# Sin3DM/Sin3DM

Hardware: AMD Instinct MI355X
Metric: DDPM-1000 triplane samples/sec @128^2 latent (higher is better)
Workload: dtype f32; 1 GPU; BASELINE configs[1]: 128^2 triplane (H,W,D)=(128,128,128), 128-ch TriplaneUNetModelSmall, DDPM-1000, batch 1 per GPU; a step = 1 denoising step; batch_per_gpu=1, parallelism=1 independent samples, prewarm_steps=150

## Files before the change

### include/sin3dm_hip.h

```cpp
#ifndef SIN3DM_HIP_H
#define SIN3DM_HIP_H

#include <stddef.h>
#include <stdint.h>

#ifdef __cplusplus
extern "C" {
#endif

#define S3D_ABI_VERSION 13
#define S3D_API __attribute__((visibility("default")))

typedef enum {
    S3D_OK = 0,
    S3D_ERR_INVALID = -1,
    S3D_ERR_MISSING = -2,
    S3D_ERR_HIP = -3,
    S3D_ERR_UNSUPPORTED = -4,
    S3D_ERR_INTERNAL = -5
} s3d_status;

S3D_API int s3d_abi_version(void);

S3D_API int s3d_set_option(const char* name, const char* value);
// ... 88 lines not shown
    const float* noise;
    const float* tables;
} s3d_known_region;
S3D_API int s3d_sampler_step_known(const s3d_sampler_args* a, const s3d_known_region* known, void* stream);
S3D_API int s3d_unet_step_film_known(s3d_unet* m, const float* film, int film_stride, int B, int H, int W, int D,
                       const s3d_sampler_args* step, const s3d_known_region* known, float* model_out, void* stream, int carry_flags);
S3D_API int s3d_sampler_renoise(const float* x_prev, const float* noise, const float* known_tables, const int64_t* t, int32_t T,
                       int64_t batch, int64_t per_sample, float* x_t, void* stream);

enum { S3D_MTAB_CX = 0, S3D_MTAB_C0, S3D_MTAB_C1, S3D_MTAB_CN, S3D_MTAB_ROWS };
typedef struct {
    const float* x0_prev;
    const float* tables;
    int32_t order;
} s3d_multistep;
S3D_API int s3d_sampler_step_multistep(const s3d_sampler_args* a, const s3d_multistep* ms, const s3d_known_region* known ,
                       void* stream);
S3D_API int s3d_unet_step_film_multistep(s3d_unet* m, const float* film, int film_stride, int B, int H, int W, int D,
                       const s3d_sampler_args* step, const s3d_multistep* ms, float* model_out, void* stream, int carry_flags);

S3D_API int s3d_op_triplane_conv(const float* const in[3], float* const out[3], int B, int C, int H, int W, int D,
                         int Cout, int ksize, int is_rollout, const float* const weight[3],
                         const float* const bias[3], void* stream);
S3D_API int s3d_op_triplane_norm_silu(const float* const in[3], float* const out[3], int B, int C, int H, int W, int D,
                              const float* const gamma[3], const float* const beta[3], void* stream);
S3D_API int s3d_op_triplane_resample(const float* const in[3], float* const out[3], int B, int C, const int hi[3],
                             const int wi[3], const int ho[3], const int wo[3], int mode, void* stream);
S3D_API int s3d_op_timestep_embed(const float* t, int B, int dim, float* out, void* stream);
S3D_API int s3d_op_triplane_resblock(const float* const in[3], float* const out[3], const float* emb, int B, int C,
                             int Cout, int H, int W, int D, int emb_dim, int use_scale_shift_norm, int is_rollout,
                             const char* const* names, const float* const* tensors, int n_tensors, void* stream);

typedef struct s3d_decoder s3d_decoder;

typedef struct {
    int32_t geo_feat_channels;
    int32_t tex_feat_channels;
    int32_t feat_channel_up;
    int32_t mlp_hidden_channels;
    int32_t mlp_hidden_layers;
    int32_t tex_channels;
} s3d_decoder_cfg;

S3D_API int s3d_decoder_create(const s3d_decoder_cfg* cfg, s3d_decoder** out);
S3D_API int s3d_decoder_create_variant(const s3d_decoder_cfg* cfg, int32_t variant, s3d_decoder** out);
S3D_API int s3d_decoder_out_channels(const s3d_decoder* d);
// ... 216 lines not shown
```

### sin3dm_amd/_lib.py

```python
from __future__ import annotations

import ctypes as C
import os

_HERE = os.path.dirname(os.path.abspath(__file__))
LIB_PATH = os.path.join(_HERE, "libsin3dm_hip.so")

c_fp = C.POINTER(C.c_float)
c_i64p = C.POINTER(C.c_int64)

ABI_VERSION = 13
TAB_ROWS = ("sqrt_recip", "sqrt_recipm1", "coef1", "coef2", "logvar", "acp", "acp_prev")
KTAB_ROWS = ("sqrt_acp_prev", "sqrt_1m_acp_prev", "sqrt_1m_beta", "sqrt_beta")
MTAB_ROWS = ("cx", "c0", "c1", "cn")
STEP_DDPM, STEP_DDIM, STEP_MEAN_ONLY = 0, 1, 2
CARRY_OUT, CARRY_IN = 1, 2
MEAN_START_X, MEAN_EPSILON = 0, 1
ERR_INVALID, ERR_MISSING, ERR_HIP, ERR_UNSUPPORTED, ERR_INTERNAL = -1, -2, -3, -4, -5
MAX_LANES = 16
MESHSDF_MAX_PAIRS = 1 << 27
RENDER_MAX_PAIRS = 1 << 27
RENDER_TILE, RENDER_SUBPIXEL, RENDER_MAX_COORD, RENDER_MAX_GRID = 16, 256, 1 << 20, 4096
IMGFEAT_INCEPTION, IMGFEAT_ALEXNET = 0, 1
RENDER_AMBIENT, RENDER_DIFFUSE = 0.35, 0.65
# ... 62 lines not shown
    "s3d_unet_current_lane": (C.c_int, [C.c_void_p]),
    "s3d_unet_forward_film": (C.c_int, [C.c_void_p, C.c_void_p, C.c_void_p, C.c_int, C.c_int, C.c_int, C.c_int, C.c_int,
                                        C.c_void_p, C.c_void_p]),
    "s3d_unet_profile": (C.c_int, [C.c_void_p, C.c_int]),
    "s3d_unet_profile_classes": (C.c_int, [C.c_void_p, C.c_int]),
    "s3d_unet_profile_read": (C.c_int, [C.c_void_p, C.POINTER(Profile)]),
    "s3d_unet_profile_kernel": (C.c_char_p, [C.c_void_p, C.c_int]),
    "s3d_sampler_step": (C.c_int, [C.POINTER(SamplerArgs), C.c_void_p]),
    "s3d_unet_step_film": (C.c_int, [C.c_void_p, C.c_void_p, C.c_int, C.c_int, C.c_int, C.c_int, C.c_int,
                                     C.POINTER(SamplerArgs), C.c_void_p, C.c_void_p]),
    "s3d_unet_step_film_carry": (C.c_int, [C.c_void_p, C.c_void_p, C.c_int, C.c_int, C.c_int, C.c_int, C.c_int,
                                           C.POINTER(SamplerArgs), C.c_void_p, C.c_void_p, C.c_int]),
    "s3d_sampler_step_known": (C.c_int, [C.POINTER(SamplerArgs), C.POINTER(KnownRegionArgs), C.c_void_p]),
    "s3d_unet_step_film_known": (C.c_int, [C.c_void_p, C.c_void_p, C.c_int, C.c_int, C.c_int, C.c_int, C.c_int,
                                           C.POINTER(SamplerArgs), C.POINTER(KnownRegionArgs), C.c_void_p, C.c_void_p, C.c_int]),
    "s3d_sampler_step_multistep": (C.c_int, [C.POINTER(SamplerArgs), C.POINTER(MultistepArgs), C.POINTER(KnownRegionArgs), C.c_void_p]),
    "s3d_unet_step_film_multistep": (C.c_int, [C.c_void_p, C.c_void_p, C.c_int, C.c_int, C.c_int, C.c_int, C.c_int,
                                               C.POINTER(SamplerArgs), C.POINTER(MultistepArgs), C.c_void_p, C.c_void_p, C.c_int]),
    "s3d_sampler_renoise": (C.c_int, [C.c_void_p, C.c_void_p, C.c_void_p, C.c_void_p, C.c_int32, C.c_int64, C.c_int64, C.c_void_p,
                                      C.c_void_p]),
    "s3d_op_triplane_conv": (C.c_int, [C.POINTER(C.c_void_p), C.POINTER(C.c_void_p), C.c_int, C.c_int, C.c_int,
                                       C.c_int, C.c_int, C.c_int, C.c_int, C.c_int, C.POINTER(C.c_void_p),
                                       C.POINTER(C.c_void_p), C.c_void_p]),
    "s3d_op_triplane_norm_silu": (C.c_int, [C.POINTER(C.c_void_p), C.POINTER(C.c_void_p), C.c_int, C.c_int, C.c_int,
                                            C.c_int, C.c_int, C.POINTER(C.c_void_p), C.POINTER(C.c_void_p),
                                            C.c_void_p]),
    "s3d_op_triplane_resample": (C.c_int, [C.POINTER(C.c_void_p), C.POINTER(C.c_void_p), C.c_int, C.c_int,
                                           C.POINTER(C.c_int), C.POINTER(C.c_int), C.POINTER(C.c_int),
                                           C.POINTER(C.c_int), C.c_int, C.c_void_p]),
    "s3d_op_timestep_embed": (C.c_int, [C.c_void_p, C.c_int, C.c_int, C.c_void_p, C.c_void_p]),
    "s3d_op_triplane_resblock": (C.c_int, [C.POINTER(C.c_void_p), C.POINTER(C.c_void_p), C.c_void_p, C.c_int, C.c_int,
                                           C.c_int, C.c_int, C.c_int, C.c_int, C.c_int, C.c_int, C.c_int,
                                           C.POINTER(C.c_char_p), C.POINTER(C.c_void_p), C.c_int, C.c_void_p]),
    "s3d_decoder_create": (C.c_int, [C.POINTER(DecoderCfg), C.POINTER(C.c_void_p)]),
    "s3d_decoder_create_variant": (C.c_int, [C.POINTER(DecoderCfg), C.c_int32, C.POINTER(C.c_void_p)]),
    "s3d_decoder_out_channels": (C.c_int, [C.c_void_p]),
    "s3d_decoder_plane_features": (C.c_int, [C.c_void_p, C.c_int, C.c_int, C.c_void_p, C.c_void_p]),
    "s3d_decoder_destroy": (None, [C.c_void_p]),
    "s3d_decoder_num_params": (C.c_int, [C.c_void_p]),
    "s3d_decoder_param_info": (C.c_int, [C.c_void_p, C.c_int, C.POINTER(C.c_char_p), c_i64p, C.POINTER(C.c_int)]),
    "s3d_decoder_set_param": (C.c_int, [C.c_void_p, C.c_char_p, C.c_void_p, c_i64p, C.c_int]),
    "s3d_decoder_prepare_triplane": (C.c_int, [C.c_void_p, C.c_void_p, C.c_void_p, C.c_void_p, C.c_int, C.c_int,
                                               C.c_int, C.c_void_p]),
    "s3d_decoder_decode_points": (C.c_int, [C.c_void_p, C.c_void_p, C.c_int64, c_fp, C.c_int, C.c_void_p,
                                            C.c_void_p]),
    "s3d_decoder_sdf_grad": (C.c_int, [C.c_void_p, C.c_void_p, C.c_int64, c_fp, C.c_int, C.c_float, C.c_float, C.c_void_p,
# ... 207 lines not shown
```

### sin3dm_amd/csrc/s3d_common.h

```cpp
#pragma once
#include <hip/hip_runtime.h>

#include <atomic>
#include <cstdarg>
#include <cstdint>
#include <cstdio>
#include <cstring>
#include <map>
#include <string>
#include <vector>

#include "../../include/sin3dm_hip.h"

namespace s3d {

void set_error(const char* fmt, ...) __attribute__((format(printf, 1, 2)));
const char* get_error();

#define S3D_HIP(call)                                                                              \
    do {                                                                                           \
        hipError_t e__ = (call);                                                                   \
        if (e__ != hipSuccess) {                                                                   \
            s3d::set_error("%s failed: %s (%s:%d)", #call, hipGetErrorString(e__), __FILE__, __LINE__); \
            return S3D_ERR_HIP;                                                                    \
// ... 160 lines not shown
void conv_note_kernel(const char* name);
const char* conv_last_kernel();
double conv_exec_fraction(ConvKind kind, const ConvArgs& a);

struct ConvW {
    size_t dense[3] = {0, 0, 0};
    size_t bias[3] = {0, 0, 0};
    size_t rrow[3] = {0, 0, 0};
    size_t rcol[3] = {0, 0, 0};
    size_t rrow_f[3] = {0, 0, 0};
    size_t rcol_f[3] = {0, 0, 0};
    size_t wino[3] = {0, 0, 0};
    size_t wino24s[3] = {0, 0, 0};
    int cin = 0, cout = 0, k = 0;
    bool rollout = false;
    bool only24_current = false;
};
size_t push(std::vector<float>& stage, const float* src, size_t n);
__host__ __device__ inline size_t rank1_frag_index(int cin, int tap, int o, int co, int c) {
    const int g = co >> 5, i = co & 31, chunk = c >> 7, cc = c & 127, w = cc >> 5, k8 = (cc >> 3) & 3, half = (cc >> 2) & 1, e = cc & 3;
    const size_t step = size_t(g * 4 + w) * (cin / 128 * 12) + chunk * 12 + tap * 4 + k8;
    return ((step * 3 + o) * 64 + half * 32 + i) * 4 + e;
}
inline size_t rank1_frag_floats(int cin, int cout) { return size_t((cout + 31) / 32) * cin * 288; }
void pack_tconv_raw(std::vector<float>& stage, const float* const W[3], const float* const bias[3], int cin, int cout,
                    int k, bool roll, ConvW& cw);

int launch_nchw_to_nhwc(const float* in, float* out, int B, int C, int h, int w, hipStream_t st);
int launch_nhwc_to_nchw(const float* in, float* out, int B, int C, int h, int w, hipStream_t st);

struct GnPartials;
bool in_conv_gn_parts(const Geo& g, int Cin, int Cout, int nparts[3]);
int launch_in_conv(const float* x, int B, int Cin, int H, int W, int D, const float* wT, const float* bias,
                   int Cout, Tri& out, hipStream_t st, const GnPartials* part = nullptr);

constexpr int kGnChunks = 256;
struct GnStats { float* mr; };
inline int gn_subgroup(int C) {
    int cg = C / 32, sg = 1;
    while (sg < 32 && cg % (sg * 2) == 0) sg *= 2;
    return sg;
}
int launch_gn_partials(const Tri& x, int B, GnPartials out, hipStream_t st);
int launch_gn_finalize(const GnPartials& part, const Geo& g, int C, int B, GnStats out, hipStream_t st);
bool gn_finalize_rider(const GnPartials& part, const Geo& g, int C, int B, GnStats out, ConvRider& r);
bool gn_partials_up_rider(const Tri& u, int B, int sg, GnPartials out, ConvRider& r);
bool gn_finalize_cat_rider(const GnPartials& pu, const GnPartials& ps, const Geo& g, int C, int B, GnStats out, ConvRider& r);
// ... 82 lines not shown
```

### sin3dm_amd/csrc/s3d_conv.hip

```cpp
#include "s3d_common.h"
#include "s3d_rank1.h"
#include "s3d_riders.h"

namespace s3d {

typedef float f32x16 __attribute__((ext_vector_type(16)));

#ifndef S3D_ABLATE
#define S3D_ABLATE 0
#endif
constexpr int KC = 32;
constexpr int LDP = KC + 4;

__device__ __forceinline__ float up2x_blend(float ly0, float ly1, float lx0, float lx1, float v00, float v01, float v10, float v11) {
    const float top = __fmaf_rn(lx1, v01, __fmul_rn(lx0, v00));
    const float bot = __fmaf_rn(lx1, v11, __fmul_rn(lx0, v10));
    return __fmaf_rn(ly1, bot, __fmul_rn(ly0, top));
}

template <int TH_, int TW_, int KH_, int KW_, int WM_, int WN_, int MTW_, int NTW_, int KS_ = 1, int PF_ = 0, bool TR_ = false>
struct ConvCfg {
    static constexpr int KS = KS_;
    static constexpr int PF = PF_;
    static constexpr bool TR = TR_;
// ... 528 lines not shown
    float* red = lds_dyn;
#pragma unroll
    for (int o = 0; o < 3; ++o)
#pragma unroll
        for (int r = 0; r < 16; ++r) red[((wid * 3 + o) * 16 + r) * 64 + lane] = q[o][r];
    __syncthreads();
    float* out = J.out + size_t(sl) * B * L * 4 * cout;
#pragma unroll
    for (int k = 0; k < 4; ++k) {
        const int it = tid + 256 * k, r = it >> 6, l = it & 63;
        float u[3];
#pragma unroll
        for (int o = 0; o < 3; ++o) {
            const float* p = red + (o * 16 + r) * 64 + l;
            u[o] = ((p[0] + p[3 * 1024]) + p[2 * 3 * 1024]) + p[3 * 3 * 1024];
        }
        const int row = mtile * 32 + (r & 3) + 8 * (r >> 2) + 4 * (l >> 5), co = g * 32 + (l & 31);
        if (row < L && co < cout) {
            float* o4 = out + (size_t(b) * L + row) * 4 * cout + co;
            o4[0] = (u[0] + u[1]) + u[2]; o4[cout] = u[1] + u[2]; o4[2 * cout] = u[0] + u[1]; o4[3 * cout] = u[1];
        }
    }
}
bool rank1b_takes(const ConvArgs& a) {
    if (a.cin % kR1Chunk != 0) return false;
    for (int j = 0; j < a.njobs; ++j) if (!a.job[j].wgt_r1f) return false;
    const int nchunks = a.cin / kR1Chunk, maxch = a.r1_slices > 1 ? (nchunks + 1) / 2 : nchunks;
    if (34 * (maxch * kR1Chunk + 4) > kR1bLdsFloats) return false;
    return opt_on(OPT_RANK1_BATCH);
}

int conv_rank1_slices(int cin) {
    return opt_on(OPT_RANK1_SLICES) && cin >= 2 * kR1Chunk && cin % kR1Chunk == 0 ? 2 : 1;
}

__global__ void k_rank1_roll_naive(ConvArgs args) {
    for (int j = 0; j < args.njobs; ++j) {
        const ConvJob& J = args.job[j];
        const int L = J.w, cout = args.cout, cin = args.cin, nt = (cout + 7) / 8;
        const long long n = (long long)args.B * L * cout;
        for (long long i = (long long)blockIdx.x * blockDim.x + threadIdx.x; i < n; i += (long long)gridDim.x * blockDim.x) {
            const int co = int(i % cout), pos = int((i / cout) % L), b = int(i / cout / L);
            float u[3] = {0.f, 0.f, 0.f};
            for (int o = 0; o < 3; ++o)
                for (int t = 0; t < 3; ++t) {
                    const int q = pos + t - 1;
// ... 7 lines not shown
        }
    }
}

int launch_rank1(ConvArgs& a, hipStream_t st, bool roll3) {
    S3D_CHECK(a.njobs >= 1 && a.njobs <= kMaxConvJobs && a.cin % KC == 0, S3D_ERR_INVALID, "rank1: bad arguments");
    S3D_CHECK(a.r1_slices <= 1 || (roll3 && !conv_use_naive() && a.r1_slices == 2 && a.cin % kR1Chunk == 0 && a.cin >= 2 * kR1Chunk), S3D_ERR_INVALID, "rank1: two K slices of whole 128-channel chunks");
    if (conv_use_naive()) {
        if (!roll3) return launch_conv_naive(CONV_1x3_VEC, a, st);
        hipLaunchKernelGGL(k_rank1_roll_naive, dim3(512), dim3(256), 0, st, a);
        S3D_HIP(hipGetLastError());
        return 0;
    }
    if (roll3 && rank1b_takes(a)) {
        int blocks = 0;
        for (int j = 0; j < a.njobs; ++j) {
            ConvJob& J = a.job[j];
            J.tiles_x = J.tiles_per_img = (J.w + 31) / 32;
            J.n_tiles_n = (a.cout + 31) / 32;
            J.block_begin = blocks;
            blocks += J.tiles_per_img * a.B * J.n_tiles_n * (a.r1_slices > 1 ? a.r1_slices : 1);
        }
        if (!blocks) return 0;
        conv_note_kernel("k_rank1b (three-tap rollout tables, fragment-order weights)");
        hipLaunchKernelGGL(k_rank1b, dim3(blocks), dim3(256), kR1bLdsFloats * sizeof(float), st, a);
        S3D_HIP(hipGetLastError());
        return 0;
    }
    const bool pair_ok = opt_on(OPT_RANK1_BATCH);
    const int ns = roll3 && pair_ok && a.B >= 2 ? 2 : 1;
    int blocks = 0;
    for (int j = 0; j < a.njobs; ++j) {
        ConvJob& J = a.job[j];
        J.tiles_x = J.tiles_per_img = (J.w + 31) / 32;
        J.n_tiles_n = roll3 ? (a.cout + 7) / 8 : (a.cout + 31) / 32;
        J.block_begin = blocks;
        blocks += J.tiles_per_img * J.n_tiles_n * ((a.B + ns - 1) / ns) * (roll3 && a.r1_slices > 1 ? a.r1_slices : 1);
    }
    if (!blocks) return 0;
    conv_note_kernel(roll3 ? "k_rank1<true> (three-tap rollout tables)" : "k_rank1<false>");
    constexpr size_t lds1 = kR1LdsFloats * sizeof(float), lds2 = lds1 + 34 * kR1Ld * sizeof(float);
    if (ns == 2) {
        static std::atomic<unsigned long long> opted{0};
        S3D_TRY(ensure_dynamic_lds(reinterpret_cast<const void*>(&k_rank1<true, 2>), int(lds2), opted));
        hipLaunchKernelGGL((k_rank1<true, 2>), dim3(blocks), dim3(256), lds2, st, a);
    } else if (roll3) hipLaunchKernelGGL(k_rank1<true>, dim3(blocks), dim3(256), 0, st, a);
// ... 147 lines not shown
```

### sin3dm_amd/csrc/s3d_ops.hip

```cpp
#include "s3d_model.h"

using namespace s3d;

namespace {

struct Scratch {
    std::vector<void*> ptrs;
    ~Scratch() { for (void* p : ptrs) (void)hipFree(p); }
    template <class T>
    int alloc(T** out, size_t n) {
        void* p = nullptr;
        S3D_HIP(hipMalloc(&p, std::max<size_t>(n, 1) * sizeof(T)));
        ptrs.push_back(p);
        *out = static_cast<T*>(p);
        return 0;
    }
};

int tri_from_nchw(Scratch& sc, const float* const in[3], int B, int C, const Geo& g, Tri& t, hipStream_t st) {
    t.C = C; t.g = g;
    for (int p = 0; p < 3; ++p) {
        S3D_TRY(sc.alloc(&t.p[p], size_t(B) * C * g.h[p] * g.w[p]));
        S3D_TRY(launch_nchw_to_nhwc(in[p], t.p[p], B, C, g.h[p], g.w[p], st));
    }
    return 0;
}
int tri_alloc(Scratch& sc, int B, int C, const Geo& g, Tri& t) {
    t.C = C; t.g = g;
    for (int p = 0; p < 3; ++p) S3D_TRY(sc.alloc(&t.p[p], size_t(B) * C * g.h[p] * g.w[p]));
    return 0;
}
int tri_to_nchw(const Tri& t, int B, float* const out[3], hipStream_t st) {
    for (int p = 0; p < 3; ++p) S3D_TRY(launch_nhwc_to_nchw(t.p[p], out[p], B, t.C, t.g.h[p], t.g.w[p], st));
    return 0;
}

}

extern "C" {

int s3d_op_triplane_conv(const float* const in[3], float* const out[3], int B, int C, int H, int W, int D, int Cout,
                         int ksize, int is_rollout, const float* const weight[3], const float* const bias[3],
                         void* stream) {
    S3D_CHECK(in && out && weight && bias, S3D_ERR_INVALID, "op_triplane_conv: null argument");
    S3D_CHECK(ksize == 1 || ksize == 3, S3D_ERR_INVALID, "op_triplane_conv: kernel size %d", ksize);
    S3D_CHECK(!is_rollout || ksize == 3, S3D_ERR_INVALID, "op_triplane_conv: rollout needs a 3x3 kernel");
    S3D_CHECK(C % 32 == 0, S3D_ERR_INVALID, "op_triplane_conv: C=%d must be a multiple of 32", C);
    hipStream_t st = static_cast<hipStream_t>(stream);
    Scratch sc;
    const Geo g = Geo::from_hwd(H, W, D);
    Tri x, y, o;
    S3D_TRY(tri_from_nchw(sc, in, B, C, g, x, st));
    S3D_TRY(tri_alloc(sc, B, Cout, g, o));

    std::vector<float> stage;
    ConvW cw;
    pack_tconv_raw(stage, weight, bias, C, Cout, ksize, is_rollout != 0, cw);
    float* wdev = nullptr;
    S3D_TRY(sc.alloc(&wdev, stage.size()));
    S3D_HIP(hipMemcpyAsync(wdev, stage.data(), stage.size() * sizeof(float), hipMemcpyHostToDevice, st));

    float* tab_row[3] = {nullptr, nullptr, nullptr};
    float* tab_col[3] = {nullptr, nullptr, nullptr};
    if (is_rollout) {
        S3D_TRY(tri_alloc(sc, B, C, g, y));
        MeanPartials mp; MeanVecs mv;
        for (int p = 0; p < 3; ++p) {
            const int h = g.h[p], w = g.w[p];
            const int ntc = (w + kActCols - 1) / kActCols, ntr = (h + kActRows - 1) / kActRows;
            S3D_TRY(sc.alloc(&mp.rowpart[p], size_t(B) * ntc * h * C));
            S3D_TRY(sc.alloc(&mp.colpart[p], size_t(B) * ntr * w * C));
            S3D_TRY(sc.alloc(&mv.rowmean[p], size_t(B) * h * C));
            S3D_TRY(sc.alloc(&mv.colmean[p], size_t(B) * w * C));
            S3D_TRY(sc.alloc(&tab_row[p], size_t(B) * h * 4 * Cout));
            S3D_TRY(sc.alloc(&tab_col[p], size_t(B) * w * 4 * Cout));
        }
        ActArgs aa; memset(&aa, 0, sizeof aa);
        S3D_TRY(launch_gn_act(x, B, GnStats{nullptr}, aa, y, &mp, st));
        S3D_TRY(launch_means_finalize(g, C, B, mp, mv, st));
        ConvArgs ca; memset(&ca, 0, sizeof ca);
        ca.B = B; ca.cin = C; ca.cout = Cout; ca.njobs = 6;
        const float* rowvec[3] = {mv.rowmean[1], mv.rowmean[0], mv.colmean[0]};
        const float* colvec[3] = {mv.rowmean[2], mv.colmean[2], mv.colmean[1]};
        for (int p = 0; p < 3; ++p) {
            ConvJob& jr = ca.job[2 * p];
            jr.in = rowvec[p]; jr.wgt = wdev + cw.rrow[p]; jr.out = tab_row[p]; jr.h = 1; jr.w = g.h[p];
            jr.wgt_r1f = cw.rrow_f[p] ? wdev + cw.rrow_f[p] : nullptr;
            ConvJob& jc = ca.job[2 * p + 1];
            jc.in = colvec[p]; jc.wgt = wdev + cw.rcol[p]; jc.out = tab_col[p]; jc.h = 1; jc.w = g.w[p];
            jc.wgt_r1f = cw.rcol_f[p] ? wdev + cw.rcol_f[p] : nullptr;
        }
        S3D_TRY(launch_conv(CONV_1x3_ROLL, ca, st));
    }
    ConvArgs ca; memset(&ca, 0, sizeof ca);
    ca.B = B; ca.cin = C; ca.cout = Cout; ca.njobs = 3;
    for (int p = 0; p < 3; ++p) {
        ConvJob& J = ca.job[p];
        J.in = x.p[p]; J.wgt = wdev + cw.dense[p]; J.bias = wdev + cw.bias[p];
        J.wgt_wino = ksize == 3 ? wdev + cw.wino[p] : nullptr;
        J.wgt_wino24s = ksize == 3 && cw.wino24s[p] ? wdev + cw.wino24s[p] : nullptr;
        J.rrow = tab_row[p]; J.rcol = tab_col[p]; J.out = o.p[p]; J.h = g.h[p]; J.w = g.w[p];
    }
    S3D_TRY(launch_conv(ksize == 3 ? CONV_3x3 : CONV_1x1, ca, st));
    S3D_TRY(tri_to_nchw(o, B, out, st));
    S3D_HIP(hipStreamSynchronize(st));
    return 0;
}

int s3d_op_triplane_norm_silu(const float* const in[3], float* const out[3], int B, int C, int H, int W, int D,
                              const float* const gamma[3], const float* const beta[3], void* stream) {
    S3D_CHECK(in && out && gamma && beta, S3D_ERR_INVALID, "op_triplane_norm_silu: null argument");
    hipStream_t st = static_cast<hipStream_t>(stream);
    Scratch sc;
    const Geo g = Geo::from_hwd(H, W, D);
    Tri x, y;
    S3D_TRY(tri_from_nchw(sc, in, B, C, g, x, st));
    S3D_TRY(tri_alloc(sc, B, C, g, y));
    GnPartials part;
    S3D_TRY(sc.alloc(&part.p, size_t(B) * 3 * kGnChunks * 64));
    part.maxparts = kGnChunks; part.nsub = 32;
    for (int p = 0; p < 3; ++p) part.nparts[p] = kGnChunks;
    GnStats stats;
    S3D_TRY(sc.alloc(&stats.mr, size_t(B) * 3 * 64));
    ActArgs aa; memset(&aa, 0, sizeof aa);
    for (int p = 0; p < 3; ++p) {
        float *gd, *bd;
        S3D_TRY(sc.alloc(&gd, C)); S3D_TRY(sc.alloc(&bd, C));
        S3D_HIP(hipMemcpyAsync(gd, gamma[p], C * sizeof(float), hipMemcpyHostToDevice, st));
        S3D_HIP(hipMemcpyAsync(bd, beta[p], C * sizeof(float), hipMemcpyHostToDevice, st));
        aa.gamma[p] = gd; aa.beta[p] = bd;
// ... 108 lines not shown
```

### sin3dm_amd/csrc/s3d_pack.hip

```cpp
#include "s3d_model.h"

namespace s3d {



constexpr int kPackItems = 1024;
__device__ __forceinline__ void repack_item(const PackDesc& d, long long i, const float* __restrict__ flat, float* __restrict__ wbuf,
                                            float* __restrict__ tbuf) {
    const float* W = flat + d.src;
    float* dst = (d.to_tbuf ? tbuf : wbuf) + d.dst;
    const int cout = d.cout, ctot = d.ctot, cin = d.cin, taps = d.taps;
    switch (d.kind) {
        case PK_COPY: dst[i] = W[i]; break;
        case PK_TRANS2D: {
            const int c = int(i / cout), o = int(i % cout);
            dst[i] = W[(size_t)o * cin + c];
            break;
        }
        case PK_DENSE: {
            const int c = int(i % cin), co = int(i / cin);
            const float* src = W + ((size_t)co * ctot + c) * taps;
            for (int t = 0; t < taps; ++t) dst[((size_t)t * cout + co) * cin + c] = src[t];
            break;
        }
// ... 85 lines not shown
        }
        case PK_RANK1: {
            const int c = int(i % cin), co = int(i / cin);
            const int n3 = (cout + 7) / 8 * 24;
            const float* src = W + ((size_t)co * ctot + d.slot * cin + c) * 9;
#pragma unroll
            for (int t = 0; t < 3; ++t)
#pragma unroll
                for (int o = 0; o < 3; ++o) {
                    const int kh = d.col_varying ? o : t, kw = d.col_varying ? t : o;
                    dst[((size_t)t * n3 + (co / 8) * 24 + o * 8 + (co & 7)) * cin + c] = src[kh * 3 + kw];
                }
            break;
        }
        case PK_RANK1F: {
            const int c = int(i % cin), co = int(i / cin);
            const float* src = W + ((size_t)co * ctot + d.slot * cin + c) * 9;
#pragma unroll
            for (int t = 0; t < 3; ++t)
#pragma unroll
                for (int o = 0; o < 3; ++o) {
                    const int kh = d.col_varying ? o : t, kw = d.col_varying ? t : o;
                    dst[rank1_frag_index(cin, t, o, co, c)] = src[kh * 3 + kw];
                }
            break;
        }
        case PK_RANK1_BWD: {
            const int co = int(i % cout), c = int(i / cout);
            const float* src = W + ((size_t)co * ctot + d.slot * cin + c) * 9;
#pragma unroll
            for (int tap = 0; tap < 3; ++tap)
#pragma unroll
                for (int j = 0; j < 3; ++j) {
                    const int dr = d.col_varying ? j : 2 - tap, dc = d.col_varying ? 2 - tap : j;
                    dst[((size_t)tap * cin + c) * (3 * cout) + j * cout + co] = src[dr * 3 + dc];
                }
            break;
        }
    }
}
__global__ __launch_bounds__(256) void k_repack(const PackDesc* __restrict__ descs, int ndesc, const float* __restrict__ flat,
                                                float* __restrict__ wbuf, float* __restrict__ tbuf) {
    const int* block_desc = reinterpret_cast<const int*>(descs + ndesc);
    const PackDesc d = descs[block_desc[blockIdx.x]];
    const long long i0 = (long long)(int(blockIdx.x) - d.block_begin) * kPackItems + threadIdx.x;
#pragma unroll
// ... 163 lines not shown
```

### sin3dm_amd/csrc/s3d_runtime.hip

```cpp
#include "s3d_common.h"
#include <atomic>

namespace s3d {

static thread_local char g_err[1024] = "";

void set_error(const char* fmt, ...) {
    va_list ap;
    va_start(ap, fmt);
    vsnprintf(g_err, sizeof g_err, fmt, ap);
    va_end(ap);
}
const char* get_error() { return g_err; }

int DevBuf::reserve(size_t bytes) {
    if (bytes <= cap) return 0;
    release();
    S3D_HIP(hipMalloc(&p, bytes));
    cap = bytes;
    return 0;
}
void DevBuf::release() {
    if (p) (void)hipFree(p);
    p = nullptr;
    cap = 0;
}
int workspace_overrun(const char* what, size_t run_peak, size_t measured) {
    if (run_peak <= measured) return 0;
    set_error("%s: the run pass took %zu bytes of workspace, the measuring pass found %zu (internal error: the workspace key "
              "misses something the allocations depend on)", what, run_peak, measured);
    return S3D_ERR_INTERNAL;
}
int upload(DevBuf& dst, const void* host, size_t bytes) {
    S3D_TRY(dst.reserve(bytes));
    S3D_HIP(hipMemcpy(dst.p, host, bytes, hipMemcpyHostToDevice));
    return 0;
}

static std::atomic<int> g_opt[OPT_COUNT];
static std::atomic<int> g_opt_state[OPT_COUNT];
static std::atomic<long long> g_opt_gen{0};
long long opt_generation() { return g_opt_gen.load(std::memory_order_acquire); }
static int parse_opt(int o, const char* v) {
    if (o == OPT_CONV_IMPL) return strcmp(v, "naive") == 0 ? 1 : 0;
    char* end = nullptr;
    const long n = strtol(v, &end, 10);
    if (end == v || *end) return kOptUnset;
    return (o == OPT_WINO ? n == 0 || n == 4 || n == 24 : n == 0 || n == 1) ? int(n) : kOptUnset;
}
static const char* opt_values(int o) { return o == OPT_WINO ? "0, 4 or 24" : "0 or 1"; }
int opt(Opt o) {
    if (g_opt_state[o].load(std::memory_order_acquire) == 0) {
        const std::string env = std::string("S3D_") + kOptNames[o];
        const char* e = getenv(env.c_str());
        int expect = 0;
        const int v = e ? parse_opt(o, e) : kOptUnset;
        if (g_opt_state[o].compare_exchange_strong(expect, -1, std::memory_order_acq_rel)) {
            g_opt[o].store(v, std::memory_order_relaxed);
            g_opt_state[o].store(1, std::memory_order_release);
        } else while (g_opt_state[o].load(std::memory_order_acquire) < 0) {}
    }
    return g_opt[o].load(std::memory_order_relaxed);
}
static int find_opt(const char* name) {
    if (!name) return -1;
    if (strncmp(name, "S3D_", 4) == 0) name += 4;
    for (int o = 0; o < OPT_COUNT; ++o) if (strcmp(name, kOptNames[o]) == 0) return o;
    return -1;
}
static std::atomic<int> g_riders{-1};
bool riders_enabled() {
    int v = g_riders.load(std::memory_order_acquire);
    if (v < 0) {
// ... 122 lines not shown
```

### sin3dm_amd/csrc/s3d_unet.hip

```cpp
#include "s3d_model.h"


namespace s3d {

static void add_lin(std::vector<ParamSpec>& s, const std::string& p, int o, int i) {
    s.push_back({p + ".weight", {o, i}});
    s.push_back({p + ".bias", {o}});
}
static void add_tconv(std::vector<ParamSpec>& s, const std::string& p, int cin, int cout, int k, bool roll) {
    for (int i = 0; i < 3; ++i) {
        s.push_back({p + ".conv_" + kPlane[i] + ".weight", {cout, roll ? 3 * cin : cin, k, k}});
        s.push_back({p + ".conv_" + kPlane[i] + ".bias", {cout}});
    }
}
static void add_tnorm(std::vector<ParamSpec>& s, const std::string& p, int c) {
    for (int i = 0; i < 3; ++i) {
        s.push_back({p + ".norm_" + kPlane[i] + ".weight", {c}});
        s.push_back({p + ".norm_" + kPlane[i] + ".bias", {c}});
    }
}
static void add_resblock(std::vector<ParamSpec>& s, const std::string& p, int c, int cout, int ted, bool ssn, bool roll) {
    add_tnorm(s, p + ".in_layers.0", c);
    add_tconv(s, p + ".in_layers.2", c, cout, 3, roll);
    add_lin(s, p + ".emb_layers.1", ssn ? 2 * cout : cout, ted);
// ... 66 lines not shown
            for (int co = 0; co < cout; ++co)
                for (int c = 0; c < cin; ++c) d[(size_t(t) * cout + co) * cin + c] = W[(size_t(co) * ctot + c) * taps + t];
        if (k == 3) cw.wino[p] = pack_wino_weights(stage, W, cout, ctot, cin);
        if (k == 3 && cin % 32 == 0) {
            cw.wino24s[p] = pack_wino24s_weights(stage, W, cout, ctot, cin);
        }
        if (!roll) continue;
        const bool a_is_col = (p == 0);
        for (int slot = 1; slot <= 2; ++slot) {
            const bool col_varying = (slot == 1) ? a_is_col : !a_is_col;
            const int n3 = (cout + 7) / 8 * 24;
            size_t off = push(stage, nullptr, size_t(3) * n3 * cin);
            float* r = stage.data() + off;
            std::fill(r, r + size_t(3) * n3 * cin, 0.f);
            for (int t = 0; t < 3; ++t)
                for (int o = 0; o < 3; ++o)
                    for (int co = 0; co < cout; ++co) {
                        const int kh = col_varying ? o : t, kw = col_varying ? t : o;
                        float* dst = r + (size_t(t) * n3 + (co / 8) * 24 + o * 8 + (co & 7)) * cin;
                        for (int c = 0; c < cin; ++c) dst[c] = W[(size_t(co) * ctot + slot * cin + c) * 9 + kh * 3 + kw];
                    }
            if (col_varying) cw.rcol[p] = off; else cw.rrow[p] = off;
            if (cin % 128 == 0) {
                const size_t off_f = push(stage, nullptr, rank1_frag_floats(cin, cout));
                float* f = stage.data() + off_f;
                std::fill(f, f + rank1_frag_floats(cin, cout), 0.f);
                const float* r2 = stage.data() + off;
                for (int t = 0; t < 3; ++t)
                    for (int o = 0; o < 3; ++o)
                        for (int co = 0; co < cout; ++co) {
                            const float* src = r2 + (size_t(t) * n3 + (co / 8) * 24 + o * 8 + (co & 7)) * cin;
                            for (int c = 0; c < cin; ++c) f[rank1_frag_index(cin, t, o, co, c)] = src[c];
                        }
                if (col_varying) cw.rcol_f[p] = off_f; else cw.rrow_f[p] = off_f;
            }
        }
    }
}
static void pack_tconv(s3d_unet* m, const std::string& prefix, int cin, int cout, int k, bool roll, ConvW& cw) {
    const float* W[3]; const float* bv[3];
    for (int p = 0; p < 3; ++p) {
        W[p] = H(m, prefix + ".conv_" + kPlane[p] + ".weight").data();
        bv[p] = H(m, prefix + ".conv_" + kPlane[p] + ".bias").data();
    }
    pack_tconv_raw(m->stage, W, bv, cin, cout, k, roll, cw);
}
static void pack_norm(s3d_unet* m, const std::string& prefix, int c, NormW& nw) {
    for (int p = 0; p < 3; ++p) {
        nw.gamma[p] = push(m->stage, H(m, prefix + ".norm_" + kPlane[p] + ".weight").data(), c);
        nw.beta[p] = push(m->stage, H(m, prefix + ".norm_" + kPlane[p] + ".bias").data(), c);
    }
}

int pack_all(s3d_unet* m) {
    for (const auto& sp : m->specs)
// ... 444 lines not shown
```

### sin3dm_amd/ops.py

```python
from __future__ import annotations

import ctypes as C

import torch as th

from . import _lib


def _prep(fm):
    fm = [f.contiguous().float() for f in fm]
    for f in fm:
        _lib.require_gpu(f)
    B, Cc, H, W = fm[0].shape
    D = fm[1].shape[-1]
    assert fm[1].shape == (B, Cc, H, D) and fm[2].shape == (B, Cc, W, D)
    return fm, B, Cc, H, W, D


def _host3(ts):
    ts = [t.detach().to("cpu", th.float32).contiguous() for t in ts]
    return ts, (C.c_void_p * 3)(*[C.c_void_p(t.data_ptr()) for t in ts])


def triplane_conv(fm, weights, biases, is_rollout):
    fm, B, Cc, H, W, D = _prep(fm)
    cout, _, k, _ = weights[0].shape
    outs = [th.empty((B, cout) + tuple(f.shape[-2:]), device=f.device) for f in fm]
    wk, wp = _host3(weights)
    bk, bp = _host3(biases)
    _lib.check(_lib.load().s3d_op_triplane_conv(_lib.ptr3(fm), _lib.ptr3(outs), B, Cc, H, W, D, cout, k,
                                                int(bool(is_rollout)), wp, bp, _lib.stream_ptr()))
    return outs


def triplane_norm_silu(fm, gammas, betas):
    fm, B, Cc, H, W, D = _prep(fm)
    outs = [th.empty_like(f) for f in fm]
    gk, gp = _host3(gammas)
    bk, bp = _host3(betas)
    _lib.check(_lib.load().s3d_op_triplane_norm_silu(_lib.ptr3(fm), _lib.ptr3(outs), B, Cc, H, W, D, gp, bp,
                                                     _lib.stream_ptr()))
    return outs


def _resample(fm, sizes, mode):
    fm = [f.contiguous().float() for f in fm]
    B, Cc = fm[0].shape[:2]
    hi = (C.c_int * 3)(*[f.shape[-2] for f in fm])
    wi = (C.c_int * 3)(*[f.shape[-1] for f in fm])
    ho = (C.c_int * 3)(*[s[0] for s in sizes])
    wo = (C.c_int * 3)(*[s[1] for s in sizes])
    outs = [th.empty((B, Cc) + tuple(s), device=f.device) for f, s in zip(fm, sizes)]
    _lib.check(_lib.load().s3d_op_triplane_resample(_lib.ptr3(fm), _lib.ptr3(outs), B, Cc, hi, wi, ho, wo, mode,
                                                    _lib.stream_ptr()))
    return outs
# ... 30 lines not shown
```

Measured before the change: 1.194 samples/s.

## Add narrow-tile rank-1 rollout conv kernel for batch-1 with second fragment layout

Result: no change. 1.203 samples/s, median of 6 (+0.8%).

```diff
diff --git a/include/sin3dm_hip.h b/include/sin3dm_hip.h
--- a/include/sin3dm_hip.h
+++ b/include/sin3dm_hip.h
@@ -134,6 +134,10 @@
 S3D_API int s3d_op_triplane_conv(const float* const in[3], float* const out[3], int B, int C, int H, int W, int D,
                          int Cout, int ksize, int is_rollout, const float* const weight[3],
                          const float* const bias[3], void* stream);
+S3D_API int s3d_op_triplane_conv_ex(const float* const in[3], float* const out[3], int B, int C, int H, int W, int D,
+                         int Cout, int ksize, int is_rollout, const float* const weight[3], const float* const bias[3],
+                         int r1_slices, float* tables, long long tables_floats, void* stream);
+S3D_API const char* s3d_op_last_conv_kernel(int which);
 S3D_API int s3d_op_triplane_norm_silu(const float* const in[3], float* const out[3], int B, int C, int H, int W, int D,
                               const float* const gamma[3], const float* const beta[3], void* stream);
 S3D_API int s3d_op_triplane_resample(const float* const in[3], float* const out[3], int B, int C, const int hi[3],
diff --git a/sin3dm_amd/_lib.py b/sin3dm_amd/_lib.py
--- a/sin3dm_amd/_lib.py
+++ b/sin3dm_amd/_lib.py
@@ -108,6 +108,10 @@
     "s3d_op_triplane_conv": (C.c_int, [C.POINTER(C.c_void_p), C.POINTER(C.c_void_p), C.c_int, C.c_int, C.c_int,
                                        C.c_int, C.c_int, C.c_int, C.c_int, C.c_int, C.POINTER(C.c_void_p),
                                        C.POINTER(C.c_void_p), C.c_void_p]),
+    "s3d_op_triplane_conv_ex": (C.c_int, [C.POINTER(C.c_void_p), C.POINTER(C.c_void_p), C.c_int, C.c_int, C.c_int,
+                                          C.c_int, C.c_int, C.c_int, C.c_int, C.c_int, C.POINTER(C.c_void_p),
+                                          C.POINTER(C.c_void_p), C.c_int, C.c_void_p, C.c_longlong, C.c_void_p]),
+    "s3d_op_last_conv_kernel": (C.c_char_p, [C.c_int]),
     "s3d_op_triplane_norm_silu": (C.c_int, [C.POINTER(C.c_void_p), C.POINTER(C.c_void_p), C.c_int, C.c_int, C.c_int,
                                             C.c_int, C.c_int, C.POINTER(C.c_void_p), C.POINTER(C.c_void_p),
                                             C.c_void_p]),
diff --git a/sin3dm_amd/csrc/s3d_common.h b/sin3dm_amd/csrc/s3d_common.h
--- a/sin3dm_amd/csrc/s3d_common.h
+++ b/sin3dm_amd/csrc/s3d_common.h
@@ -206,7 +206,13 @@
     const size_t step = size_t(g * 4 + w) * (cin / 128 * 12) + chunk * 12 + tap * 4 + k8;
     return ((step * 3 + o) * 64 + half * 32 + i) * 4 + e;
 }
-inline size_t rank1_frag_floats(int cin, int cout) { return size_t((cout + 31) / 32) * cin * 288; }
+__host__ __device__ inline size_t rank1_frag_floats(int cin, int cout) { return size_t((cout + 31) / 32) * cin * 288; }
+__host__ __device__ inline size_t rank1c_frag_index(int cin, int tap, int o, int co, int c) {
+    const int g = co >> 3, col = o * 8 + (co & 7), chunk = c >> 7, cc = c & 127, w = cc >> 5, k8 = (cc >> 3) & 3, half = (cc >> 2) & 1, e = cc & 3;
+    const size_t step = size_t(g * 4 + w) * (cin / 128 * 12) + chunk * 12 + tap * 4 + k8;
+    return (step * 64 + half * 32 + col) * 4 + e;
+}
+__host__ __device__ inline size_t rank1c_frag_floats(int cin, int cout) { return size_t((cout + 7) / 8) * cin * 96; }
 void pack_tconv_raw(std::vector<float>& stage, const float* const W[3], const float* const bias[3], int cin, int cout,
                     int k, bool roll, ConvW& cw);
 
diff --git a/sin3dm_amd/csrc/s3d_conv.hip b/sin3dm_amd/csrc/s3d_conv.hip
--- a/sin3dm_amd/csrc/s3d_conv.hip
+++ b/sin3dm_amd/csrc/s3d_conv.hip
@@ -574,6 +574,98 @@
         }
     }
 }
+__global__ __launch_bounds__(256) void k_rank1c(ConvArgs args) {
+    extern __shared__ __attribute__((aligned(16))) float lds_dyn[];
+    int bid = blockIdx.x;
+    if ((gridDim.x & 7) == 0) bid = (bid & 7) * int(gridDim.x >> 3) + (bid >> 3);
+    int j = 0;
+#pragma unroll
+    for (int k = 1; k < kMaxConvJobs; ++k) j += (k < args.njobs && bid >= args.job[k].block_begin) ? 1 : 0;
+    const ConvJob& J = args.job[j];
+    int local = bid - J.block_begin;
+    const int L = J.w, cin = args.cin, cout = args.cout, B = args.B;
+    const int mtile = local % J.tiles_per_img; local /= J.tiles_per_img;
+    const int b = local % B; local /= B;
+    const int g = local % J.n_tiles_n, sl = local / J.n_tiles_n;
+    const int nchunks = cin / kR1Chunk;
+    int chunk0 = 0, nch = nchunks;
+    if (args.r1_slices > 1) { const int first = (nchunks + 1) / 2; chunk0 = sl ? first : 0; nch = sl ? nchunks - first : first; }
+    const int csl = nch * kR1Chunk, ld = csl + 4;
+    const int tid = threadIdx.x, lane = tid & 63, wid = __builtin_amdgcn_readfirstlane(tid >> 6), i = lane & 31, half = lane >> 5;
+    const int nsteps = nch * 12;
+    const r1_f32x4* pf = reinterpret_cast<const r1_f32x4*>(J.wgt_r1f + rank1_frag_floats(cin, cout)) + (size_t(g * 4 + wid) * (nchunks * 12) + chunk0 * 12) * 64 + lane;
+    constexpr int D = 12;
+    r1_f32x4 ring[D];
+    int pf_s = 0;
+    auto prefetch = [&](int slot) {
+        ring[slot] = ((r1_gf4ptr)(uintptr_t)pf)[0];
+        ++pf_s;
+        pf += pf_s < nsteps ? 64 : 0;
+    };
+#pragma unroll
+    for (int d = 0; d < D; ++d) prefetch(d);
+    {
+        const int q4 = csl / 4, items = 34 * q4;
+        const float* vb = J.in + (size_t(b) * L) * cin + chunk0 * kR1Chunk;
+        const r1_f32x4 zero4 = {0.f, 0.f, 0.f, 0.f};
+        for (int it0 = tid; it0 < items; it0 += 256 * 5) {
+            r1_f32x4 v[5];
+#pragma unroll
+            for (int u = 0; u < 5; ++u) {
+                const int it = it0 + 256 * u, row = it / q4, q = it - row * q4, pos = mtile * 32 - 1 + row;
+                const bool ok = it < items && pos >= 0 && pos < L;
+                v[u] = ((r1_gf4ptr)(uintptr_t)(vb + size_t(ok ? pos : 0) * cin + (ok ? q : 0) * 4))[0];
+                if (!ok) v[u] = zero4;
+            }
+#pragma unroll
+            for (int u = 0; u < 5; ++u) {
+                const int it = it0 + 256 * u, row = it / q4, q = it - row * q4;
+                if (it < items) *reinterpret_cast<r1_f32x4*>(lds_dyn + row * ld + q * 4) = v[u];
+            }
+        }
+    }
+    __syncthreads();
+    r1_f32x16 q;
+#pragma unroll
+    for (int r = 0; r < 16; ++r) q[r] = 0.f;
+    const float* Ab = lds_dyn + i * ld + half * 4 + wid * 32;
+    for (int ch = 0; ch < nch; ++ch) {
+        const float* Ac = Ab + ch * kR1Chunk;
+#pragma unroll
+        for (int st = 0; st < 12; ++st) {
+            const int tap = st >> 2, k8 = st & 3;
+            const r1_f32x4 a4 = *reinterpret_cast<const r1_f32x4*>(Ac + tap * ld + k8 * 8);
+            const r1_f32x4 b4 = ring[st];
+            __builtin_amdgcn_sched_barrier(0);
+#pragma unroll
+            for (int e = 0; e < 4; ++e) q = __builtin_amdgcn_mfma_f32_32x32x2f32(a4[e], b4[e], q, 0, 0, 0);
+            __builtin_amdgcn_sched_barrier(0);
+            prefetch(st);
+            __builtin_amdgcn_sched_barrier(0);
+        }
+    }
+    __syncthreads();
+    float* red = lds_dyn;
+#pragma unroll
+    for (int r = 0; r < 16; ++r) red[(wid * 16 + r) * 64 + lane] = q[r];
+    __syncthreads();
+    float* out = J.out + size_t(sl) * B * L * 4 * cout;
+    {
+        const int r = tid >> 4, hf = (tid >> 3) & 1, c8 = tid & 7;
+        float u[3];
+#pragma unroll
+        for (int o = 0; o < 3; ++o) {
+            const float* p = red + r * 64 + hf * 32 + o * 8 + c8;
+            u[o] = ((p[0] + p[1024]) + p[2 * 1024]) + p[3 * 1024];
+        }
+        const int row = mtile * 32 + (r & 3) + 8 * (r >> 2) + 4 * hf, co = g * 8 + c8;
+        if (row < L && co < cout) {
+            float* o4 = out + (size_t(b) * L + row) * 4 * cout + co;
+            o4[0] = (u[0] + u[1]) + u[2]; o4[cout] = u[1] + u[2]; o4[2 * cout] = u[0] + u[1]; o4[3 * cout] = u[1];
+        }
+    }
+}
+constexpr int kR1cRedFloats = 4 * 16 * 64;
 bool rank1b_takes(const ConvArgs& a) {
     if (a.cin % kR1Chunk != 0) return false;
     for (int j = 0; j < a.njobs; ++j) if (!a.job[j].wgt_r1f) return false;
@@ -627,6 +719,27 @@
             blocks += J.tiles_per_img * a.B * J.n_tiles_n * (a.r1_slices > 1 ? a.r1_slices : 1);
         }
         if (!blocks) return 0;
+        {
+            const int cus = device_cus(), mode = opt(OPT_RANK1_BATCH);
+            const int nchunks = a.cin / kR1Chunk, maxch = a.r1_slices > 1 ? (nchunks + 1) / 2 : nchunks;
+            long long blocks_c = 0;
+            for (int j = 0; j < a.njobs; ++j) blocks_c += (long long)a.job[j].tiles_per_img * a.B * ((a.cout + 7) / 8) * (a.r1_slices > 1 ? a.r1_slices : 1);
+            const long long chain_b = (blocks + cus - 1) / cus * 144LL * maxch, chain_c = (blocks_c + cus - 1) / cus * 48LL * maxch;
+            if (mode != 2 && blocks_c < (1LL << 30) && (mode == 3 || (a.B == 1 && chain_c < chain_b))) {
+                blocks = 0;
+                for (int j = 0; j < a.njobs; ++j) {
+                    ConvJob& J = a.job[j];
+                    J.n_tiles_n = (a.cout + 7) / 8;
+                    J.block_begin = blocks;
+                    blocks += J.tiles_per_img * a.B * J.n_tiles_n * (a.r1_slices > 1 ? a.r1_slices : 1);
+                }
+                const size_t lds = std::max<size_t>(size_t(34) * (maxch * kR1Chunk + 4), kR1cRedFloats) * sizeof(float);
+                conv_note_kernel("k_rank1c (three-tap rollout tables, fragment-order weights, one accumulator per wave)");
+                hipLaunchKernelGGL(k_rank1c, dim3(blocks), dim3(256), lds, st, a);
+                S3D_HIP(hipGetLastError());
+                return 0;
+            }
+        }
         conv_note_kernel("k_rank1b (three-tap rollout tables, fragment-order weights)");
         hipLaunchKernelGGL(k_rank1b, dim3(blocks), dim3(256), kR1bLdsFloats * sizeof(float), st, a);
         S3D_HIP(hipGetLastError());
diff --git a/sin3dm_amd/csrc/s3d_ops.hip b/sin3dm_amd/csrc/s3d_ops.hip
--- a/sin3dm_amd/csrc/s3d_ops.hip
+++ b/sin3dm_amd/csrc/s3d_ops.hip
@@ -37,16 +37,20 @@
 
 }
 
-extern "C" {
-
-int s3d_op_triplane_conv(const float* const in[3], float* const out[3], int B, int C, int H, int W, int D, int Cout,
-                         int ksize, int is_rollout, const float* const weight[3], const float* const bias[3],
-                         void* stream) {
-    S3D_CHECK(in && out && weight && bias, S3D_ERR_INVALID, "op_triplane_conv: null argument");
-    S3D_CHECK(ksize == 1 || ksize == 3, S3D_ERR_INVALID, "op_triplane_conv: kernel size %d", ksize);
-    S3D_CHECK(!is_rollout || ksize == 3, S3D_ERR_INVALID, "op_triplane_conv: rollout needs a 3x3 kernel");
-    S3D_CHECK(C % 32 == 0, S3D_ERR_INVALID, "op_triplane_conv: C=%d must be a multiple of 32", C);
-    hipStream_t st = static_cast<hipStream_t>(stream);
+static thread_local std::string t_op_kernel[2];
+
+static int triplane_conv_op(const float* const in[3], float* const out[3], int B, int C, int H, int W, int D, int Cout,
+                            int ksize, int is_rollout, const float* const weight[3], const float* const bias[3],
+                            int r1_slices, float* tables, long long tables_floats, const char* who, hipStream_t st) {
+    S3D_CHECK(in && out && weight && bias, S3D_ERR_INVALID, "%s: null argument", who);
+    S3D_CHECK(ksize == 1 || ksize == 3, S3D_ERR_INVALID, "%s: kernel size %d", who, ksize);
+    S3D_CHECK(!is_rollout || ksize == 3, S3D_ERR_INVALID, "%s: rollout needs a 3x3 kernel", who);
+    S3D_CHECK(C % 32 == 0, S3D_ERR_INVALID, "%s: C=%d must be a multiple of 32", who, C);
+    const bool w24 = ksize == 3 && conv_wino24_channels(C, Cout) && !conv_use_naive();
+    const int nsl = r1_slices == 2 ? 2 : 1;
+    S3D_CHECK(r1_slices >= 0 && r1_slices <= 2 && (nsl == 1 || (is_rollout && w24 && C % 128 == 0 && C >= 256)), S3D_ERR_INVALID,
+              "%s: two K slices need a rollout convolution of the mixed Winograd kernel over at least two whole 128-channel chunks", who);
+    S3D_CHECK(!tables || is_rollout, S3D_ERR_INVALID, "%s: only a rollout convolution has tables", who);
     Scratch sc;
     const Geo g = Geo::from_hwd(H, W, D);
     Tri x, y, o;
@@ -65,6 +69,11 @@
     if (is_rollout) {
         S3D_TRY(tri_alloc(sc, B, C, g, y));
         MeanPartials mp; MeanVecs mv;
+        size_t tab_total = 0;
+        for (int p = 0; p < 3; ++p) tab_total += size_t(nsl) * B * (g.h[p] + g.w[p]) * 4 * Cout;
+        S3D_CHECK(!tables || tables_floats == (long long)tab_total, S3D_ERR_INVALID, "%s: the tables take %zu floats, not %lld", who, tab_total, tables_floats);
+        float* tab = tables;
+        if (!tab) S3D_TRY(sc.alloc(&tab, tab_total));
         for (int p = 0; p < 3; ++p) {
             const int h = g.h[p], w = g.w[p];
             const int ntc = (w + kActCols - 1) / kActCols, ntr = (h + kActRows - 1) / kActRows;
@@ -72,14 +81,15 @@
             S3D_TRY(sc.alloc(&mp.colpart[p], size_t(B) * ntr * w * C));
             S3D_TRY(sc.alloc(&mv.rowmean[p], size_t(B) * h * C));
             S3D_TRY(sc.alloc(&mv.colmean[p], size_t(B) * w * C));
-            S3D_TRY(sc.alloc(&tab_row[p], size_t(B) * h * 4 * Cout));
-            S3D_TRY(sc.alloc(&tab_col[p], size_t(B) * w * 4 * Cout));
+            tab_row[p] = tab; tab += size_t(nsl) * B * h * 4 * Cout;
+            tab_col[p] = tab; tab += size_t(nsl) * B * w * 4 * Cout;
         }
         ActArgs aa; memset(&aa, 0, sizeof aa);
         S3D_TRY(launch_gn_act(x, B, GnStats{nullptr}, aa, y, &mp, st));
         S3D_TRY(launch_means_finalize(g, C, B, mp, mv, st));
         ConvArgs ca; memset(&ca, 0, sizeof ca);
         ca.B = B; ca.cin = C; ca.cout = Cout; ca.njobs = 6;
+        ca.r1_slices = nsl == 2 ? 2 : 0;
         const float* rowvec[3] = {mv.rowmean[1], mv.rowmean[0], mv.colmean[0]};
         const float* colvec[3] = {mv.rowmean[2], mv.colmean[2], mv.colmean[1]};
         for (int p = 0; p < 3; ++p) {
@@ -91,9 +101,11 @@
             jc.wgt_r1f = cw.rcol_f[p] ? wdev + cw.rcol_f[p] : nullptr;
         }
         S3D_TRY(launch_conv(CONV_1x3_ROLL, ca, st));
-    }
+        t_op_kernel[1] = conv_last_kernel();
+    } else t_op_kernel[1].clear();
     ConvArgs ca; memset(&ca, 0, sizeof ca);
     ca.B = B; ca.cin = C; ca.cout = Cout; ca.njobs = 3;
+    ca.r1_slices = nsl == 2 ? 2 : 0;
     for (int p = 0; p < 3; ++p) {
         ConvJob& J = ca.job[p];
         J.in = x.p[p]; J.wgt = wdev + cw.dense[p]; J.bias = wdev + cw.bias[p];
@@ -102,10 +114,29 @@
         J.rrow = tab_row[p]; J.rcol = tab_col[p]; J.out = o.p[p]; J.h = g.h[p]; J.w = g.w[p];
     }
     S3D_TRY(launch_conv(ksize == 3 ? CONV_3x3 : CONV_1x1, ca, st));
+    t_op_kernel[0] = conv_last_kernel();
     S3D_TRY(tri_to_nchw(o, B, out, st));
     S3D_HIP(hipStreamSynchronize(st));
     return 0;
 }
+
+extern "C" {
+
+int s3d_op_triplane_conv(const float* const in[3], float* const out[3], int B, int C, int H, int W, int D, int Cout,
+                         int ksize, int is_rollout, const float* const weight[3], const float* const bias[3],
+                         void* stream) {
+    return triplane_conv_op(in, out, B, C, H, W, D, Cout, ksize, is_rollout, weight, bias, 0, nullptr, 0, "op_triplane_conv",
+                            static_cast<hipStream_t>(stream));
+}
+
+int s3d_op_triplane_conv_ex(const float* const in[3], float* const out[3], int B, int C, int H, int W, int D, int Cout,
+                            int ksize, int is_rollout, const float* const weight[3], const float* const bias[3],
+                            int r1_slices, float* tables, long long tables_floats, void* stream) {
+    return triplane_conv_op(in, out, B, C, H, W, D, Cout, ksize, is_rollout, weight, bias, r1_slices, tables, tables_floats,
+                            "op_triplane_conv_ex", static_cast<hipStream_t>(stream));
+}
+
+const char* s3d_op_last_conv_kernel(int which) { return which == 0 || which == 1 ? t_op_kernel[which].c_str() : ""; }
 
 int s3d_op_triplane_norm_silu(const float* const in[3], float* const out[3], int B, int C, int H, int W, int D,
                               const float* const gamma[3], const float* const beta[3], void* stream) {
diff --git a/sin3dm_amd/csrc/s3d_pack.hip b/sin3dm_amd/csrc/s3d_pack.hip
--- a/sin3dm_amd/csrc/s3d_pack.hip
+++ b/sin3dm_amd/csrc/s3d_pack.hip
@@ -131,6 +131,7 @@
                 for (int o = 0; o < 3; ++o) {
                     const int kh = d.col_varying ? o : t, kw = d.col_varying ? t : o;
                     dst[rank1_frag_index(cin, t, o, co, c)] = src[kh * 3 + kw];
+                    dst[rank1_frag_floats(cin, cout) + rank1c_frag_index(cin, t, o, co, c)] = src[kh * 3 + kw];
                 }
             break;
         }
diff --git a/sin3dm_amd/csrc/s3d_runtime.hip b/sin3dm_amd/csrc/s3d_runtime.hip
--- a/sin3dm_amd/csrc/s3d_runtime.hip
+++ b/sin3dm_amd/csrc/s3d_runtime.hip
@@ -46,9 +46,12 @@
     char* end = nullptr;
     const long n = strtol(v, &end, 10);
     if (end == v || *end) return kOptUnset;
+    if (o == OPT_RANK1_BATCH) return n >= 0 && n <= 3 ? int(n) : kOptUnset;
     return (o == OPT_WINO ? n == 0 || n == 4 || n == 24 : n == 0 || n == 1) ? int(n) : kOptUnset;
 }
-static const char* opt_values(int o) { return o == OPT_WINO ? "0, 4 or 24" : "0 or 1"; }
+static const char* opt_values(int o) {
+    return o == OPT_WINO ? "0, 4 or 24" : (o == OPT_RANK1_BATCH ? "0, 1, 2 or 3" : "0 or 1");
+}
 int opt(Opt o) {
     if (g_opt_state[o].load(std::memory_order_acquire) == 0) {
         const std::string env = std::string("S3D_") + kOptNames[o];
diff --git a/sin3dm_amd/csrc/s3d_unet.hip b/sin3dm_amd/csrc/s3d_unet.hip
--- a/sin3dm_amd/csrc/s3d_unet.hip
+++ b/sin3dm_amd/csrc/s3d_unet.hip
@@ -112,15 +112,16 @@
                     }
             if (col_varying) cw.rcol[p] = off; else cw.rrow[p] = off;
             if (cin % 128 == 0) {
-                const size_t off_f = push(stage, nullptr, rank1_frag_floats(cin, cout));
+                const size_t nf = rank1_frag_floats(cin, cout), nfc = rank1c_frag_floats(cin, cout);
+                const size_t off_f = push(stage, nullptr, nf + nfc);
                 float* f = stage.data() + off_f;
-                std::fill(f, f + rank1_frag_floats(cin, cout), 0.f);
+                std::fill(f, f + nf + nfc, 0.f);
                 const float* r2 = stage.data() + off;
                 for (int t = 0; t < 3; ++t)
                     for (int o = 0; o < 3; ++o)
                         for (int co = 0; co < cout; ++co) {
                             const float* src = r2 + (size_t(t) * n3 + (co / 8) * 24 + o * 8 + (co & 7)) * cin;
-                            for (int c = 0; c < cin; ++c) f[rank1_frag_index(cin, t, o, co, c)] = src[c];
+                            for (int c = 0; c < cin; ++c) { f[rank1_frag_index(cin, t, o, co, c)] = src[c]; f[nf + rank1c_frag_index(cin, t, o, co, c)] = src[c]; }
                         }
                 if (col_varying) cw.rcol_f[p] = off_f; else cw.rrow_f[p] = off_f;
             }
diff --git a/sin3dm_amd/ops.py b/sin3dm_amd/ops.py
--- a/sin3dm_amd/ops.py
+++ b/sin3dm_amd/ops.py
@@ -31,6 +31,26 @@
     _lib.check(_lib.load().s3d_op_triplane_conv(_lib.ptr3(fm), _lib.ptr3(outs), B, Cc, H, W, D, cout, k,
                                                 int(bool(is_rollout)), wp, bp, _lib.stream_ptr()))
     return outs
+
+
+def triplane_conv_ex(fm, weights, biases, is_rollout, r1_slices=1, tables=False):
+    fm, B, Cc, H, W, D = _prep(fm)
+    cout, _, k, _ = weights[0].shape
+    outs = [th.empty((B, cout) + tuple(f.shape[-2:]), device=f.device) for f in fm]
+    wk, wp = _host3(weights)
+    bk, bp = _host3(biases)
+    tab = None
+    if tables:
+        tab = th.empty((2 if r1_slices == 2 else 1) * B * 4 * cout * 2 * (H + W + D), device=fm[0].device)
+    _lib.check(_lib.load().s3d_op_triplane_conv_ex(
+        _lib.ptr3(fm), _lib.ptr3(outs), B, Cc, H, W, D, cout, k, int(bool(is_rollout)), wp, bp, int(r1_slices),
+        tab.data_ptr() if tab is not None else None, tab.numel() if tab is not None else 0, _lib.stream_ptr()))
+    return outs, tab
+
+
+def last_conv_kernels():
+    lib = _lib.load()
+    return lib.s3d_op_last_conv_kernel(0).decode(), lib.s3d_op_last_conv_kernel(1).decode()
 
 
 def triplane_norm_silu(fm, gammas, betas):
```
